# facebook/transform360

Hardware: NVIDIA H100
Metric: Mpixels/s 8K equirect->cubemap bicubic (input-plane pixels consumed per second) (higher is better)
Workload: dtype u8

## Files before the change

include/transform360_b200.h:

```cpp
#ifndef TRANSFORM360_B200_EXT_H
#define TRANSFORM360_B200_EXT_H

#include "Transform360/VideoFrameTransformHandler.h"

#ifdef __cplusplus
extern "C" {
#endif

typedef struct T360HostPlan T360HostPlan;

T360HostPlan* T360B200_hostPlanCreate(const FrameTransformContext* ctx, int inputWidth, int inputHeight,
                                      int outputWidth, int outputHeight);
#define T360_BORDER_WRAP 3
#define T360_BORDER_TRANSPARENT 5
T360HostPlan* T360B200_hostPlanCreateFromWarp(const FrameTransformContext* ctx, const float* map, int mapWidth, int mapHeight,
                                              int inputWidth, int inputHeight, int border);
void T360B200_hostPlanDestroy(T360HostPlan* plan);
int T360B200_hostPlanInfo(const T360HostPlan* plan, int info[6]);
const float* T360B200_hostPlanMap(const T360HostPlan* plan);
const int32_t* T360B200_hostPlanSamples(const T360HostPlan* plan);
int T360B200_hostPlanGather(T360HostPlan* plan, int info[10], const int32_t** jobs, const int32_t** records,
                            const uint32_t** compact);
int T360B200_hostPlanPoleCaps(T360HostPlan* plan, int info[4], const int32_t** capJobs, const uint32_t** capRecords,
                              const int32_t** launchJobs);
int T360B200_dealLanes(int interpolationAlg, int n, const int32_t* phases, int32_t* laneOf, int32_t* copyOf);
int T360B200_weightImage(int interpolationAlg, const uint8_t** image);
int T360B200_hostPlanBlurLists(T360HostPlan* const* plans, int numPlans, int width, int height, int layout[15],
                               const uint8_t** image);
int T360B200_hostPlanSegment(const T360HostPlan* plan, int i, int rect[4], int numTaps[2], const float** kx,
                             const float** ky);
int T360B200_remapTable(int interpolationAlg, const int16_t** table);

int T360B200_generateMapFromWarp(VideoFrameTransform* transform, const float* map, int mapWidth, int mapHeight, int inputWidth,
                                 int inputHeight, int border, int transformMatPlaneIndex);
int T360B200_remapFrameAsync(VideoFrameTransform* transform, int numPlanes, const float* const* deviceMaps, const int* mapPitches,
                             int border, const uint8_t* const* deviceInputs, uint8_t* const* deviceOutputs, const int* inputWidths,
                             const int* inputHeights, const int* inputPitches, const int* outputWidths, const int* outputHeights,
                             const int* outputPitches, void* cudaStream);

int T360B200_transformFramePlaneAsync(VideoFrameTransform* transform, const uint8_t* deviceInput,
                                      uint8_t* deviceOutput, int inputWidth, int inputHeight, int inputPitch,
                                      int outputWidth, int outputHeight, int outputPitch,
                                      int transformMatPlaneIndex, void* cudaStream);
int T360B200_transformFrameAsync(VideoFrameTransform* transform, int numPlanes, const uint8_t* const* deviceInputs,
                                 uint8_t* const* deviceOutputs, const int* inputWidths, const int* inputHeights,
                                 const int* inputPitches, const int* outputWidths, const int* outputHeights,
                                 const int* outputPitches, void* cudaStream);
// ... 67 lines not shown
```

profiles/trace_frame.py:

```python
#!/usr/bin/env python
import sys
from pathlib import Path

import numpy as np
import torch

sys.path.insert(0, str(Path(__file__).resolve().parents[1]))
import transform360_b200 as t360
from bench import CONFIGS
from transform360_b200 import synth
from transform360_b200.stream import FrameTransformer, StreamSpec

KINDS = {0: "class0", 1: "class1", 3: "share-stay", 4: "share", 5: "nop", 7: "seam", 8: "pole-cap", 9: "border"}


def main():
    name = sys.argv[1] if len(sys.argv) > 1 else "cfg2"
    cfg = CONFIGS[name]
    dev = torch.device("cuda", 0)
    torch.cuda.set_device(0)
    ctx = t360.make_context(**dict(cfg["ov"], enable_low_pass_filter=0))
    spec = StreamSpec(cfg["inp"][0], cfg["inp"][1], cfg["out"][0], cfg["out"][1])
    ft = FrameTransformer(ctx, spec)
    pitch = lambda w: (w + 255) // 256 * 256
    ring = 5
    d_in = [[synth.noise_plane_torch(*spec.plane_dims(p)[:2], plane=p, frame=f, device=dev, pitch=pitch(spec.plane_dims(p)[0])) for p in range(3)]
            for f in range(ring)]
    d_out = [torch.zeros((spec.plane_dims(p)[3], pitch(spec.plane_dims(p)[2])), dtype=torch.uint8, device=dev) for p in range(3)]
    calls = [ft.frame_call([(t.data_ptr(), t.stride(0)) for t in fr], [(t.data_ptr(), t.stride(0)) for t in d_out]) for fr in d_in]
    stream = torch.cuda.Stream(device=dev)
    torch.cuda.synchronize()
    for i in range(6):
        calls[i % ring](stream.cuda_stream)
    torch.cuda.synchronize()
    ft.vft.debug_trace(True)
    calls[1](stream.cuda_stream)
# ... 25 lines not shown
```

transform360_b200/csrc/gather_frame.cu:

```cuda
#include "gather_common.cuh"

#include <cuda.h>

#include <algorithm>
#include <cstring>
#include <utility>

namespace t360 {

namespace {

template <class F, int... I>
__device__ __forceinline__ void staticForImpl(F&& f, std::integer_sequence<int, I...>) {
  (f(std::integral_constant<int, I>{}), ...);
}
template <int N, class F>
__device__ __forceinline__ void staticFor(F&& f) {
  staticForImpl(f, std::make_integer_sequence<int, N>{});
}

template <int IMM>
__device__ __forceinline__ uint32_t ldsWordImm(uint32_t addr) {
  uint32_t v;
  asm volatile("ld.shared.u32 %0, [%1+%2];" : "=r"(v) : "r"(addr), "n"(IMM));
// ... 177 lines not shown
  });
}

template <int K, int PITCH, int VS>
__device__ __forceinline__ void computeTileJob(const PlaneView& pv, uint32_t stageAddr, int outX, int outY, const uint4& rec,
                                               uint32_t wAddr, int warp) {
  static_assert(PITCH % 4 == 0, "");
  const int y0 = outY + warp * kTilePatchH;
  const int dstPitch = pv.dstPitch, dstW = pv.dstW, dstH = pv.dstH;
  uint8_t* const dstRow = pv.dst + (size_t)y0 * dstPitch + outX;
  const uint32_t words[4] = {rec.x, rec.y, rec.z, rec.w};
  staticFor<kRowsPerPatchStep>([&](auto J) {
    constexpr int j = decltype(J)::value;
    const uint32_t w = words[j];
    const int col = kTilePatchW * j + ((int)(w >> 16) & (kTilePatchW - 1)), row = (int)(w >> 19) & (kTilePatchH - 1);
    if (!(w & kRecordSkip) && outX + col < dstW && y0 + row < dstH) {
      const uint32_t rowAddr = stageAddr + (w & 0x7ffcu);
      const int sh = (int)(w << 3);
      RowBytes<K> W[K];
      staticFor<K>([&](auto R) { W[decltype(R)::value] = loadRow<K, decltype(R)::value * PITCH>(rowAddr, sh); });
      const int acc = foldPixel<K, VS>(W, wAddr, (w >> 17) & kSlotFieldMask);
      dstRow[(size_t)row * dstPitch + col] = (uint8_t)biasedToByte(acc);
    }
  });
}

template <int K, int PITCH, int VS>
__device__ __forceinline__ void computeCapJob(const PlaneView& pv, uint32_t stageAddr, uint32_t recAddr, int steps, uint32_t wAddr,
                                              int warp, int lane) {
  static_assert(PITCH % 4 == 0, "");
  for (int s = warp; s < steps; s += kGroupWarps) {
    const uint2 r = ldsVec2Imm<0>(recAddr + s * kCapStepBytes + lane * 8);
    if (r.x & kRecordSkip) continue;
    const uint32_t rowAddr = stageAddr + (r.x & 0x7ffcu);
    const int sh = (int)(r.x << 3);
    RowBytes<K> W[K];
    staticFor<K>([&](auto R) { W[decltype(R)::value] = loadRow<K, decltype(R)::value * PITCH>(rowAddr, sh); });
    const int acc = foldPixel<K, VS>(W, wAddr, (r.x >> 17) & kSlotFieldMask);
    pv.dst[(size_t)(r.y >> 16) * pv.dstPitch + (r.y & 0xffffu)] = (uint8_t)biasedToByte(acc);
  }
}

template <int K, int VS>
__device__ __forceinline__ void computeBorderJob(const PlaneView& pv, uint32_t recAddr, int n, const unsigned char* wsmem, int warp, int lane) {
  SrcView sv;
  sv.bytes = pv.src;
// ... 184 lines not shown
      if constexpr (K >= 4) {
        const uint32_t mine = rec + 128 + warp * shareWarpRecordBytes(K);
        uint4 r[shareRows(K) / 8];
#pragma unroll
        for (int b = 0; b < shareRows(K) / 8; ++b) r[b] = ldsVec(mine + b * 512 + lane * 16);
        const uint32_t header = ldsWord(mine + shareRows(K) / 8 * 512 + lane * 4);
        uint8_t* dst = pv.dst + (size_t)(outY + (warp >> 1) * shareRows(K)) * pv.dstPitch + (outX + (warp & 1) * 32 + (int)(header >> kRecordColumnShift));
        if (kind == kJobShare) computeShareJob<K, stageBoxW(K, 2), VS, shareRows(K), false>(dst, pv.dstPitch, boxAddr + st * kStage, r, header, wAddr);
        else computeShareJob<K, stageBoxW(K, 2), VS, shareRows(K), true>(dst, pv.dstPitch, boxAddr + st * kStage, r, header, wAddr);
      }
    } else if (kind == kJobClass0) {
      uint4 r;
      const int quad = ((int)h.x & kJobQuadMask) - 1;
      if (quad < 0) {
        r = ldsVec(rec + 128 + warp * 512 + lane * 16);
      } else {
        r = make_uint4(kRecordSkip, kRecordSkip, kRecordSkip, kRecordSkip);
        if ((warp >> 2) == (quad >> 1)) {
          const uint2 v = ldsVec2Imm<0>(rec + 128 + (warp & 3) * 256 + lane * 8);
          if (quad & 1) { r.z = v.x; r.w = v.y; } else { r.x = v.x; r.y = v.y; }
        }
      }
      computeTileJob<K, stageBoxW(K, 0), VS>(pv, boxAddr + st * kStage, outX, outY, r, wAddr, warp);
    } else if (kind == kJobClass1) {
      computeTileJob<K, stageBoxW(K, 1), VS>(pv, boxAddr + st * kStage, outX, outY, ldsVec(rec + 128 + warp * 512 + lane * 16), wAddr, warp);
    } else if (kind == kJobSeam) {
      {
        uint4* a = reinterpret_cast<uint4*>(groupBase + st * kStage);
        const uint4* b = reinterpret_cast<const uint4*>(groupBase + (st + 1) * kStage);
        for (int i = warp * 32 + lane; i < (int)(kBox0 / 16); i += kGroupThreads) {
          uint4 x = a[i];
          const uint4 y = b[i];
          x.x |= y.x; x.y |= y.y; x.z |= y.z; x.w |= y.w;
          a[i] = x;
        }
        asm volatile("fence.proxy.async.shared::cta;" ::: "memory");
      }
      groupBarrier(group);
      computeTileJob<K, stageBoxW(K, 0), VS>(pv, boxAddr + st * kStage, outX, outY, ldsVec(rec + 128 + warp * 512 + lane * 16), wAddr, warp);
    } else if (kind == kJobCap) {
      computeCapJob<K, stageBoxW(K, 0), VS>(pv, boxAddr + st * kStage, rec + 128, (int)h.x, wAddr, warp, lane);
    } else if (kind == kJobBorder) {
      computeBorderJob<K, VS>(pv, rec + 128, (int)h.x, wsmem, warp, lane);
    }
    __syncwarp();
    if (lane == 0) mbarArrive(empty + st);
// ... 69 lines not shown
```

transform360_b200/csrc/gather_plan.cpp:

```cpp
#include "gather_plan.h"

#include <algorithm>
#include <climits>
#include <cstdint>
#include <cstring>
#include <stdexcept>
#include <thread>
#include <utility>

namespace t360 {
namespace {

template <class F>
void parallelRanges(int n, size_t workPerItem, F fn) {
  unsigned nt = std::thread::hardware_concurrency();
  if (nt == 0) nt = 1;
  if (nt > 32) nt = 32;
  if (static_cast<size_t>(n) * workPerItem < (1u << 16)) nt = 1;
  const int chunk = (n + static_cast<int>(nt) - 1) / static_cast<int>(nt);
  std::vector<std::thread> pool;
  for (unsigned t = 1; t < nt; ++t) {
    const int b = static_cast<int>(t) * chunk, e = std::min(n, b + chunk);
    if (b < e) pool.emplace_back(fn, b, e);
  }
// ... 604 lines not shown
  coverPoleCaps(h, cls, tilesX, tilesY, pixelJobs);
  for (PixelJob& pj : pixelJobs) {
    const int kind = (pj.job.outY >> kJobKindShift) & kJobKindMask;
    pj.job.recordOffset = static_cast<int>(offset / 16);
    offset += jobRecordBytes(k, kind, pj.job.outX);
    g.capJobs.push_back(pj.job);
    g.capRecords.insert(g.capRecords.end(), pj.words.begin(), pj.words.end());
    ++(kind == kJobCap ? g.numCap : g.numBorder);
  }

  std::vector<int> launch;
  for (size_t i = 0; i < g.jobs.size(); ++i)
    if (((g.jobs[i].outY >> kJobKindShift) & kJobKindMask) != kJobGeneral) launch.push_back(static_cast<int>(i));
  for (size_t i = 0; i < g.capJobs.size(); ++i) launch.push_back(-1 - static_cast<int>(i));
  auto jobOf = [&](int i) -> const GatherJob& { return i >= 0 ? g.jobs[i] : g.capJobs[-1 - i]; };
  std::stable_sort(launch.begin(), launch.end(), [&](int a, int b) { return jobLaunchRank(jobOf(a)) < jobLaunchRank(jobOf(b)); });
  for (int i : launch) {
    g.launchJobs.push_back(jobOf(i));
    g.launchNeedRows.push_back(i >= 0 ? needRows[i] : pixelJobs[-1 - i].needRows);
    g.launchRects.push_back(i >= 0 ? rects[i] : pixelJobs[-1 - i].rect);
  }
}

}
```

transform360_b200/csrc/gather_plan.h:

```cpp
#pragma once

#include <cstdint>
#include <vector>

#include "host_plan.h"
#include "kernels.cuh"

namespace t360 {

struct JobRect {
  int x0, y0, x1, y1;
};

struct GatherPlan {
  int tilesPerRow = 0, tileRows = 0, tileH = 0;
  std::vector<int2> records;
  std::vector<GatherJob> jobs;
  std::vector<uint32_t> compact;
  std::vector<GatherJob> capJobs;
  std::vector<uint32_t> capRecords;
  std::vector<GatherJob> launchJobs;
  std::vector<int> launchNeedRows;
  std::vector<JobRect> launchRects;
  int numStaged[2] = {}, numSeam = 0, numGeneral = 0, numShare = 0, numCap = 0, numBorder = 0;
  int totalStaged() const { return numSeam + numShare + numStaged[0] + numStaged[1] + numCap; }
};

void buildGatherPlan(const HostPlan& h, bool stageTiles, GatherPlan& g);

inline int jobLaunchRank(const GatherJob& job) {
  switch ((job.outY >> kJobKindShift) & kJobKindMask) {
    case kJobBorder: case kJobGeneral: return 0;
    case kJobSeam: return 1;
    case kJobClass1: return 2;
    case kJobCap: return 3;
    case kJobShareStay: return 4;
    case kJobShare: return 5;
    default: return (job.outX & kJobQuadMask) ? 7 : 6;
  }
}


int dealLanes(int k, int copies, int n, const int* slot, int* laneOf, int* copyOf);

std::vector<uint8_t> buildWeightImage(int k, const int16_t* table);

}
```

transform360_b200/csrc/kernels.cuh:

```cuda
#pragma once

#include <cuda_runtime.h>

#include <cstdint>

#include "flat_view.h"
#include "oriented_view.h"

namespace t360 {

struct GatherParams {
  const uint8_t* src;
  int srcW, srcH, srcPitch;
  uint8_t* dst;
  int dstW, dstH, dstPitch;
  const int2* samples;
  int tilesPerRow;
  const int16_t* weights;
  int kernelSize;
  int transparent;
};

struct GatherJob {
  int outX, outY;
  int boxXY;
  int recordOffset;
};
constexpr int kBoxVariants = 3;
__host__ __device__ constexpr int jobBoxField(int boxX, int boxY, int variant) { return boxX | (boxY << 16) | variant; }
__host__ __device__ constexpr int jobBoxX(int boxXY) { return boxXY & 0xfff0; }
__host__ __device__ constexpr int jobBoxY(int boxXY) { return (int)((unsigned)boxXY >> 16); }
__host__ __device__ constexpr int jobBoxVariant(int boxXY) { return boxXY & 15; }
using StagedTile = GatherJob;
constexpr int kJobClass0 = 0, kJobClass1 = 1, kJobGeneral = 2, kJobShareStay = 3, kJobShare = 4, kJobNop = 5, kJobExit = 6, kJobSeam = 7,
              kJobCap = 8, kJobBorder = 9;
constexpr int kJobQuadMask = 7;
constexpr uint32_t kRecordSkip = 0x8000u;
constexpr int kJobKindShift = 24, kJobRowMask = (1 << kJobKindShift) - 1;
constexpr int kJobPlaneShift = 28, kJobKindMask = (1 << (kJobPlaneShift - kJobKindShift)) - 1;

constexpr int kGroupThreads = 256, kGroupWarps = kGroupThreads / 32;
__host__ __device__ constexpr int gatherGroups(int k) { return k == 8 ? 2 : 3; }
#ifndef T360_CLAIM_BATCH
#define T360_CLAIM_BATCH 1
#endif
constexpr int kClaimBatch = T360_CLAIM_BATCH;
constexpr int kGatherTileW = 32, kFrameTileH = 32;
constexpr int kTilePatchW = 8, kTilePatchH = 4, kRowsPerPatchStep = 4;
constexpr int kShareW = 64;
__host__ __device__ constexpr int shareRows(int ) { return 8; }
__host__ __device__ constexpr int shareH(int k) { return 4 * shareRows(k); }
constexpr int kNumBoxClasses = 3;
__host__ __device__ constexpr int boxClassOf(int kind) { return (kind == kJobShare || kind == kJobShareStay) ? 2 : (kind == kJobClass1 ? 1 : 0); }
__host__ __device__ constexpr int stageBoxW(int , int cls) { return cls == 2 ? 192 : (cls == 0 ? 208 : 240); }
__host__ __device__ constexpr int stageBoxH(int k, int cls) {
  return k == 8 ? (cls == 2 ? 80 : (cls == 0 ? 72 : 128)) : (cls == 2 ? 72 : (cls == 0 ? 64 : 96));
}
__host__ __device__ constexpr int boxVariantRows(int k, int cls, int v) {
// ... 28 lines not shown
  return weightDiagonal(k) ? (slotFieldValue ^ (vector * kDiagonalStep)) : slotFieldValue + vector * weightVectorStride(k, copies);
}
__host__ __device__ constexpr int weightBankGroups(int k) { return k == 2 ? 16 : 8; }
__host__ __device__ constexpr int weightLanesPerPass(int k) { return k == 2 ? 16 : 8; }

__host__ __device__ constexpr int shareWarpRecordBytes(int k) { return shareRows(k) / 8 * 32 * 16 + 32 * 4; }
__host__ __device__ constexpr int shareJobRecordBytes(int k) { return kGroupWarps * shareWarpRecordBytes(k); }
constexpr int kTileJobRecordBytes = kGroupWarps * 32 * 16;
constexpr int kQuadJobRecordBytes = kGroupWarps / 2 * 32 * 8;
__host__ __device__ constexpr int tileJobRecordBytes(int outXField) { return (outXField & kJobQuadMask) ? kQuadJobRecordBytes : kTileJobRecordBytes; }
__host__ __device__ constexpr int stageRecordBytes(int k) {
  return 128 + (shareJobRecordBytes(k) > kTileJobRecordBytes ? shareJobRecordBytes(k) : kTileJobRecordBytes);
}
constexpr int kCapStepBytes = 32 * 8, kBorderPixelBytes = 16;
__host__ __device__ constexpr int capJobMaxSteps(int k) { return (stageRecordBytes(k) - 128) / kCapStepBytes; }
__host__ __device__ constexpr int borderJobMaxPixels(int k) { return (stageRecordBytes(k) - 128) / kBorderPixelBytes; }
__host__ __device__ constexpr int jobRecordBytes(int k, int kind, int outXField) {
  return kind == kJobShare || kind == kJobShareStay ? shareJobRecordBytes(k)
         : kind == kJobCap                          ? outXField * kCapStepBytes
         : kind == kJobBorder                       ? outXField * kBorderPixelBytes
                                                    : tileJobRecordBytes(outXField);
}
constexpr int kRecordColumnShift = 27;

constexpr int kMaxFramePlanes = 3;
struct PlaneView {
  const uint8_t* src;
  uint8_t* dst;
  const uint4* records;
  int srcW, srcH, srcPitch;
  int dstW, dstH, dstPitch;
};
struct FrameGatherParams {
  PlaneView plane[kMaxFramePlanes];
  const uint4* weightImage;
  int kernelSize, numPlanes;
};

__host__ __device__ constexpr int gatherThreads(int k) { return k == 8 ? 512 : 256; }
__host__ __device__ constexpr int gatherTileH(int k) { return gatherThreads(k) / 32 * 4; }

struct StagedParams {
  const GatherJob* tiles;
  int numTiles;
  int* claimCounter;
  unsigned long long* trace;
// ... 152 lines not shown
```

transform360_b200/csrc/video_frame_transform.cpp:

```cpp
#include <cuda.h>
#include <cuda_runtime.h>

#include <algorithm>
#include <chrono>
#include <climits>
#include <cmath>
#include <condition_variable>
#include <cstdarg>
#include <cstdio>
#include <cstdlib>
#include <cstring>
#include <map>
#include <memory>
#include <mutex>
#include <new>
#include <shared_mutex>
#include <stdexcept>
#include <string>
#include <string_view>
#include <thread>
#include <vector>

#include "host_plan.h"
#include "gather_plan.h"
// ... 1325 lines not shown
    std::lock_guard<std::mutex> lock(lazyMu_);
    auto& buf = weights_[k];
    if (!buf.ptr) {
      buf.reserve(static_cast<size_t>(1024) * k * k);
      CU(cudaMemcpy(buf.ptr, host, buf.bytes(), cudaMemcpyHostToDevice));
      const std::vector<uint8_t> image = t360::buildWeightImage(k, host);
      weightImages_[k].reserve(image.size());
      CU(cudaMemcpy(weightImages_[k].ptr, image.data(), image.size(), cudaMemcpyHostToDevice));
    }
    return buf.ptr;
  }

  DevicePlan upload(HostIndexPlan& p, const FrameTransformContext& ctx) {
    const HostPlan& h = p.host;
    DevicePlan d;
    d.inW = h.inW; d.inH = h.inH; d.outW = h.outW; d.outH = h.outH; d.mapW = h.mapW; d.mapH = h.mapH;
    d.kernelSize = h.kernelSize;
    d.transparent = h.transparentBorder;
    d.warp = h.warp;
    d.stereoFormat = ctx.input_stereo_format;
    if (d.kernelSize > 0) {
      deviceWeights(ctx.interpolation_alg);
      t360::GatherPlan& g = p.gather;
      d.tilesPerRow = g.tilesPerRow;
      d.samples.reserve(g.records.size());
      CU(cudaMemcpy(d.samples.ptr, g.records.data(), g.records.size() * sizeof(int2), cudaMemcpyHostToDevice));
      d.numStaged = g.totalStaged();
      d.numBorder = g.numBorder;
      d.numJobs = static_cast<int>(g.launchJobs.size());
      if (!g.launchJobs.empty()) {
        d.gatherJobs.reserve(g.launchJobs.size());
        CU(cudaMemcpy(d.gatherJobs.ptr, g.launchJobs.data(), g.launchJobs.size() * sizeof(GatherJob), cudaMemcpyHostToDevice));
      }
      if (!g.compact.empty() || !g.capRecords.empty()) {
        d.records.reserve(g.compact.size() + g.capRecords.size());
        if (!g.compact.empty())
          CU(cudaMemcpy(d.records.ptr, g.compact.data(), g.compact.size() * sizeof(uint32_t), cudaMemcpyHostToDevice));
        if (!g.capRecords.empty())
          CU(cudaMemcpy(d.records.ptr + g.compact.size(), g.capRecords.data(), g.capRecords.size() * sizeof(uint32_t), cudaMemcpyHostToDevice));
      }
      d.hostJobs = std::move(g.launchJobs);
      d.jobNeedRows = std::move(g.launchNeedRows);
      d.jobRects = std::move(g.launchRects);
    }
    d.lowPass = ctx.enable_low_pass_filter != 0;
    if (d.lowPass) {
// ... 696 lines not shown
}

T360_API int T360B200_generateMapFromWarp(VideoFrameTransform* t, const float* map, int mapW, int mapH, int inW, int inH, int border,
                                          int planIndex) {
  if (!t) return 0;
  return t->generateMapFromWarp(map, mapW, mapH, inW, inH, border, planIndex);
}

T360_API int VideoFrameTransform_transformFramePlane(VideoFrameTransform* transform, uint8_t* inputData,
                                                     uint8_t* outputData, int inputWidth, int inputHeight,
                                                     int inputWidthWithPadding, int outputWidth, int outputHeight,
                                                     int outputWidthWithPadding, int transformMatPlaneIndex,
                                                     int imagePlaneIndex) {
  if (!transform) return 0;
  return transform->transformFramePlane(inputData, outputData, inputWidth, inputHeight, inputWidthWithPadding,
                                        outputWidth, outputHeight, outputWidthWithPadding, transformMatPlaneIndex,
                                        imagePlaneIndex);
}

struct T360HostPlan {
  HostPlan plan;
  t360::GatherPlan gather;
  bool gatherBuilt = false;
  std::vector<uint8_t> blurImage;
};

T360_API T360HostPlan* T360B200_hostPlanCreate(const FrameTransformContext* ctx, int inW, int inH, int outW, int outH) {
  if (!ctx) return nullptr;
  std::unique_ptr<T360HostPlan> p(new (std::nothrow) T360HostPlan);
  if (!p) return nullptr;
  try {
    if (!t360::buildHostPlan(*ctx, inW, inH, outW, outH, p->plan)) return nullptr;
  } catch (const std::exception& ex) {
    std::printf("Could not build the host plan. Error: %s\n", ex.what());
    return nullptr;
  }
  return p.release();
}
T360_API T360HostPlan* T360B200_hostPlanCreateFromWarp(const FrameTransformContext* ctx, const float* map, int mapW, int mapH, int inW,
                                                       int inH, int border) {
  if (!ctx) return nullptr;
  std::unique_ptr<T360HostPlan> p(new (std::nothrow) T360HostPlan);
  if (!p) return nullptr;
  try {
    if (!t360::buildWarpHostPlan(*ctx, map, mapW, mapH, inW, inH, border, p->plan)) return nullptr;
  } catch (const std::exception& ex) {
// ... 27 lines not shown
  } catch (const std::exception& ex) {
    std::printf("Could not build the gather plan. Error: %s\n", ex.what());
    return 0;
  }
  const t360::GatherPlan& g = plan->gather;
  info[0] = g.tilesPerRow; info[1] = g.tileRows; info[2] = g.tileH; info[3] = static_cast<int>(g.jobs.size());
  info[4] = g.numStaged[0]; info[5] = g.numStaged[1]; info[6] = g.numSeam; info[7] = g.numGeneral;
  info[8] = g.numShare; info[9] = static_cast<int>(g.compact.size());
  if (jobs) *jobs = g.jobs.empty() ? nullptr : reinterpret_cast<const int32_t*>(g.jobs.data());
  if (records) *records = reinterpret_cast<const int32_t*>(g.records.data());
  if (compact) *compact = g.compact.empty() ? nullptr : g.compact.data();
  return 1;
}
T360_API int T360B200_hostPlanPoleCaps(T360HostPlan* plan, int info[4], const int32_t** capJobs, const uint32_t** capRecords,
                                       const int32_t** launchJobs) {
  int gatherInfo[10];
  if (!plan || !info || !T360B200_hostPlanGather(plan, gatherInfo, nullptr, nullptr, nullptr)) return 0;
  const t360::GatherPlan& g = plan->gather;
  info[0] = g.numCap; info[1] = g.numBorder; info[2] = static_cast<int>(g.capRecords.size());
  info[3] = static_cast<int>(g.launchJobs.size());
  if (capJobs) *capJobs = g.capJobs.empty() ? nullptr : reinterpret_cast<const int32_t*>(g.capJobs.data());
  if (capRecords) *capRecords = g.capRecords.empty() ? nullptr : g.capRecords.data();
  if (launchJobs) *launchJobs = g.launchJobs.empty() ? nullptr : reinterpret_cast<const int32_t*>(g.launchJobs.data());
  return 1;
}
T360_API int T360B200_hostPlanBlurLists(T360HostPlan* const* plans, int numPlans, int width, int height, int layout[15],
                                        const uint8_t** image) {
  if (!plans || numPlans < 1 || numPlans > t360::kMaxFramePlanes || !layout || !image) return 0;
  for (int p = 0; p < numPlans; ++p)
    if (!plans[p]) return 0;
  try {
    t360::BlurLists lists[t360::kMaxFramePlanes];
    const t360::BlurLists* planes[t360::kMaxFramePlanes];
    bool clear = false;
    for (int p = 0; p < numPlans; ++p) {
      const HostPlan& h = plans[p]->plan;
      bool c = false;
      t360::buildBlurLists(h.segments, h.taps, width > 0 ? width : h.inW, height > 0 ? height : h.inH, h.ctx.input_stereo_format, lists[p], &c);
      clear = clear || c;
      planes[p] = &lists[p];
    }
    std::vector<uint8_t>& img = plans[0]->blurImage;
    img.clear();
    const t360::BlurLayout l = t360::packBlurLists(numPlans > 1 ? t360::mergeBlurLists(planes, numPlans) : lists[0], img, img);
    const long long v[15] = {l.numStrips[0], l.numStrips[1], l.numStrips[2], l.numTiles, l.numDirect, l.numTaps, l.tileSmem, clear,
                             static_cast<long long>(l.stripAt[0]), static_cast<long long>(l.stripAt[1]), static_cast<long long>(l.stripAt[2]),
// ... 218 lines not shown
```

transform360_b200/handler.py:

```python
from __future__ import annotations

import ctypes as C
import os
from pathlib import Path

import numpy as np

PKG = Path(__file__).resolve().parent
LIB_PATH = PKG / "lib" / "libTransform360.so"

LAYOUT_CUBEMAP_32, LAYOUT_CUBEMAP_23_OFFCENTER, LAYOUT_FLAT_FIXED, LAYOUT_EQUIRECT = 0, 1, 2, 3
LAYOUT_BARREL, LAYOUT_BARREL_SPLIT, LAYOUT_EAC_32, LAYOUT_N = 4, 5, 6, 7
STEREO_FORMAT_TB, STEREO_FORMAT_LR, STEREO_FORMAT_MONO, STEREO_FORMAT_GUESS, STEREO_FORMAT_N = 0, 1, 2, 3, 4
NEAREST, LINEAR, CUBIC, LANCZOS4 = 0, 1, 2, 4
BORDER_WRAP, BORDER_TRANSPARENT = 3, 5


def _warp_map(map) -> np.ndarray:
    m = np.ascontiguousarray(map, np.float32)
    if m.ndim != 3 or m.shape[2] != 2:
        raise ValueError(f"a warp map is float32 [h][w][2] (x, y per output pixel), got shape {m.shape}")
    return m


# ... 114 lines not shown
    L.T360B200_hostPlanCreate.argtypes = [C.POINTER(FrameTransformContext)] + [ci] * 4
    L.T360B200_hostPlanCreateFromWarp.restype = vp
    L.T360B200_hostPlanCreateFromWarp.argtypes = [C.POINTER(FrameTransformContext), vp] + [ci] * 5
    L.T360B200_generateMapFromWarp.restype = ci
    L.T360B200_generateMapFromWarp.argtypes = [vp, vp] + [ci] * 6
    L.T360B200_remapFrameAsync.restype = ci
    L.T360B200_remapFrameAsync.argtypes = [vp, ci, vp, vp, ci] + [vp] * 8 + [vp]
    L.T360B200_hostPlanDestroy.restype = None
    L.T360B200_hostPlanDestroy.argtypes = [vp]
    L.T360B200_hostPlanInfo.restype = ci
    L.T360B200_hostPlanInfo.argtypes = [vp, C.POINTER(ci)]
    L.T360B200_hostPlanMap.restype = vp
    L.T360B200_hostPlanMap.argtypes = [vp]
    L.T360B200_hostPlanSamples.restype = vp
    L.T360B200_hostPlanSamples.argtypes = [vp]
    L.T360B200_hostPlanSegment.restype = ci
    L.T360B200_hostPlanSegment.argtypes = [vp, ci, C.POINTER(ci), C.POINTER(ci), C.POINTER(vp), C.POINTER(vp)]
    L.T360B200_hostPlanGather.restype = ci
    L.T360B200_hostPlanGather.argtypes = [vp, C.POINTER(ci), C.POINTER(vp), C.POINTER(vp), C.POINTER(vp)]
    L.T360B200_hostPlanPoleCaps.restype = ci
    L.T360B200_hostPlanBlurLists.restype = ci
    L.T360B200_hostPlanBlurLists.argtypes = [vp, ci, ci, ci, C.POINTER(ci), C.POINTER(vp)]
    L.T360B200_hostPlanPoleCaps.argtypes = [vp, C.POINTER(ci), C.POINTER(vp), C.POINTER(vp), C.POINTER(vp)]
    L.T360B200_weightImage.restype = ci
    L.T360B200_weightImage.argtypes = [ci, C.POINTER(vp)]
    L.T360B200_remapTable.restype = ci
    L.T360B200_remapTable.argtypes = [ci, C.POINTER(vp)]
    L.T360B200_transformFramePlaneAsync.restype = ci
    L.T360B200_transformFramePlaneAsync.argtypes = [vp, vp, vp] + [ci] * 7 + [vp]
    L.T360B200_transformFrameAsync.restype = ci
    L.T360B200_transformFrameAsync.argtypes = [vp, ci, vp, vp] + [vp] * 6 + [vp]
    L.T360B200_lowPassPlaneAsync.restype = ci
    L.T360B200_lowPassPlaneAsync.argtypes = [vp, vp, vp] + [ci] * 5 + [vp]
    L.T360B200_reconfigure.restype = ci
    L.T360B200_reconfigure.argtypes = [vp, C.POINTER(FrameTransformContext)]
    L.T360B200_reconfigureAsync.restype = ci
    L.T360B200_reconfigureAsync.argtypes = [vp, C.POINTER(FrameTransformContext)]
    L.T360B200_reconfigureWait.restype = ci
    L.T360B200_reconfigureWait.argtypes = [vp, ci]
    L.T360B200_transformFrameViewAsync.restype = ci
    L.T360B200_transformFrameViewAsync.argtypes = [vp, C.POINTER(T360View), ci, vp, vp] + [vp] * 6 + [vp]
    L.T360B200_viewSamples.restype = ci
    L.T360B200_viewSamples.argtypes = [C.POINTER(FrameTransformContext), C.POINTER(T360View)] + [ci] * 4 + [vp]
    L.T360B200_transformFrameOrientedAsync.restype = ci
    L.T360B200_transformFrameOrientedAsync.argtypes = [vp, C.POINTER(T360Orientation), ci, vp, vp] + [vp] * 6 + [vp]
    L.T360B200_orientedSamples.restype = ci
# ... 13 lines not shown
    L.T360B200_debugTraceRead.restype = C.c_ulonglong
    L.T360B200_debugTraceRead.argtypes = [vp, vp, C.c_ulonglong]
    L.T360B200_synchronize.restype = ci
    L.T360B200_synchronize.argtypes = [vp]
    L.T360B200_stream.restype = vp
    L.T360B200_stream.argtypes = [vp]
    L.T360B200_kernelLaunchCount.restype = C.c_ulonglong
    L.T360B200_planDeviceBytes.restype = C.c_ulonglong
    L.T360B200_planDeviceBytes.argtypes = [vp, ci]
    L.T360B200_planTileCounts.restype = ci
    L.T360B200_planTileCounts.argtypes = [vp, ci, C.POINTER(ci)]
    L.T360B200_deviceCount.restype = ci
    L.T360B200_version.restype = C.c_char_p
    if path is None:
        _lib = L
    return L


EXPORTED_SYMBOLS = [
    "VideoFrameTransform_new", "VideoFrameTransform_delete", "VideoFrameTransform_generateMapForPlane",
    "VideoFrameTransform_transformFramePlane", "T360B200_hostPlanCreate", "T360B200_hostPlanCreateFromWarp", "T360B200_hostPlanDestroy",
    "T360B200_generateMapFromWarp", "T360B200_remapFrameAsync",
    "T360B200_hostPlanInfo", "T360B200_hostPlanMap", "T360B200_hostPlanSamples", "T360B200_hostPlanSegment",
    "T360B200_hostPlanGather", "T360B200_hostPlanPoleCaps", "T360B200_hostPlanBlurLists", "T360B200_weightImage", "T360B200_dealLanes",
    "T360B200_remapTable", "T360B200_transformFramePlaneAsync", "T360B200_transformFrameAsync",
    "T360B200_lowPassPlaneAsync", "T360B200_reconfigure", "T360B200_reconfigureAsync", "T360B200_reconfigureWait",
    "T360B200_transformFrameViewAsync", "T360B200_viewSamples",
    "T360B200_transformFrameOrientedAsync", "T360B200_orientedSamples", "T360B200_transformFramePoseAsync", "T360B200_poseSamples",
    "T360B200_lensMap", "T360B200_transformFrameLensAsync",
    "T360B200_setPinHostPlanes", "T360B200_debugTrace", "T360B200_debugTraceRead", "T360B200_synchronize", "T360B200_stream", "T360B200_kernelLaunchCount", "T360B200_planDeviceBytes",
    "T360B200_planTileCounts", "T360B200_deviceCount", "T360B200_version",
]


class VideoFrameTransform:

    def __init__(self, ctx: FrameTransformContext):
        self._lib = load()
        self.ctx = ctx
        self._h = self._lib.VideoFrameTransform_new(C.byref(ctx))
        if not self._h:
            raise MemoryError("VideoFrameTransform_new returned NULL")

    def close(self):
        if getattr(self, "_h", None):
            self._lib.VideoFrameTransform_delete(self._h)
            self._h = None
# ... 186 lines not shown
        if not self._lib.T360B200_hostPlanGather(self._h, info, C.byref(jobs), C.byref(recs), C.byref(comp)):
            raise ValueError("T360B200_hostPlanGather failed")
        tpr, trows, th, nj = info[0], info[1], info[2], info[3]
        n = tpr * trows * th * 32 * 2
        records = np.frombuffer((C.c_int32 * n).from_address(recs.value), np.int32).reshape(tpr * trows, th, 32, 2).copy()
        j = compact = None
        if nj and jobs.value:
            j = np.frombuffer((C.c_int32 * (nj * 4)).from_address(jobs.value), np.int32).reshape(nj, 4).copy()
        if info[9] and comp.value:
            compact = np.frombuffer((C.c_uint32 * info[9]).from_address(comp.value), np.uint32).copy()
        return dict(tiles_per_row=tpr, tile_rows=trows, tile_h=th, jobs=j, records=records, compact=compact,
                    counts=dict(class0=info[4], class1=info[5], seam=info[6], general=info[7], share=info[8]))

    def pole_caps(self):
        info = (C.c_int * 4)()
        jobs, recs, launch = C.c_void_p(), C.c_void_p(), C.c_void_p()
        if not self._lib.T360B200_hostPlanPoleCaps(self._h, info, C.byref(jobs), C.byref(recs), C.byref(launch)):
            raise ValueError("T360B200_hostPlanPoleCaps failed")
        n, m = info[0] + info[1], info[3]
        as_jobs = lambda p, k: np.frombuffer((C.c_int32 * (k * 4)).from_address(p.value), np.int32).reshape(k, 4).copy() if k and p.value else np.zeros((0, 4), np.int32)
        records = np.frombuffer((C.c_uint32 * info[2]).from_address(recs.value), np.uint32).copy() if info[2] and recs.value else np.zeros(0, np.uint32)
        return dict(counts=dict(cap=info[0], border=info[1]), jobs=as_jobs(jobs, n), records=records, launch=as_jobs(launch, m))

    def blur_lists(self, *others, width=0, height=0):
        plans = (C.c_void_p * (1 + len(others)))(self._h, *[o._h for o in others])
        lay, img = (C.c_int * 15)(), C.c_void_p()
        if not self._lib.T360B200_hostPlanBlurLists(plans, len(plans), width, height, lay, C.byref(img)):
            raise ValueError("T360B200_hostPlanBlurLists failed (message on stdout)")
        image = C.string_at(img.value, lay[14]) if lay[14] else b""
        arr = lambda at, n, cols, dt: np.frombuffer(image, dt, n * cols, at).reshape(n, cols).copy()
        return dict(image=image, strips=[arr(lay[8 + c], lay[c], 9, np.int32) for c in range(3)], tiles=arr(lay[11], lay[3], 8, np.int32),
                    direct=arr(lay[12], lay[4], 8, np.int32), taps=np.frombuffer(image, np.float32, lay[5], lay[13]).copy(),
                    offsets=list(lay[8:14]), tile_smem=lay[6], needs_clear=bool(lay[7]))

    def segments(self):
        out = []
        rect, nk = (C.c_int * 4)(), (C.c_int * 2)()
        kx, ky = C.c_void_p(), C.c_void_p()
        for i in range(self.num_segments):
            assert self._lib.T360B200_hostPlanSegment(self._h, i, rect, nk, C.byref(kx), C.byref(ky))
            a = np.frombuffer((C.c_float * nk[0]).from_address(kx.value), np.float32).copy()
            b = np.frombuffer((C.c_float * nk[1]).from_address(ky.value), np.float32).copy()
            out.append((rect[0], rect[1], rect[2], rect[3], a, b))
        return out


# ... 57 lines not shown
```

Measured before the change: 720,900.

## Add tile-walk job kind reusing bicubic tap words across output rows

Adds a new job kind for bicubic class-0 tiles. Each lane keeps its 4x2 shared-memory tap words in registers across the four output rows of a patch step and reloads only the words that change: a row step, a left or right word shift, or a full reload. The host planner encodes these per-lane walk flags into the records. It also picks a lane-dealing row and weight-copy assignment that minimise a modelled count of shared-memory bank wavefronts. This cuts shared-memory loads and bank conflicts in the gather kernel, at the cost of more register pressure, extra branching and heavier plan-build work on the host.

Result: faster. 764,500, median of 6 (+6.0%).

```diff
diff --git a/include/transform360_b200.h b/include/transform360_b200.h
--- a/include/transform360_b200.h
+++ b/include/transform360_b200.h
@@ -23,6 +23,8 @@
                             const uint32_t** compact);
 int T360B200_hostPlanPoleCaps(T360HostPlan* plan, int info[4], const int32_t** capJobs, const uint32_t** capRecords,
                               const int32_t** launchJobs);
+int T360B200_hostPlanTileWalk(T360HostPlan* plan, int info[4], long long model[4], const int32_t** launchJobs,
+                              const uint32_t** records);
 int T360B200_dealLanes(int interpolationAlg, int n, const int32_t* phases, int32_t* laneOf, int32_t* copyOf);
 int T360B200_weightImage(int interpolationAlg, const uint8_t** image);
 int T360B200_hostPlanBlurLists(T360HostPlan* const* plans, int numPlans, int width, int height, int layout[15],
diff --git a/profiles/trace_frame.py b/profiles/trace_frame.py
--- a/profiles/trace_frame.py
+++ b/profiles/trace_frame.py
@@ -11,7 +11,7 @@
 from transform360_b200 import synth
 from transform360_b200.stream import FrameTransformer, StreamSpec
 
-KINDS = {0: "class0", 1: "class1", 3: "share-stay", 4: "share", 5: "nop", 7: "seam", 8: "pole-cap", 9: "border"}
+KINDS = {0: "class0", 1: "class1", 3: "share-stay", 4: "share", 5: "nop", 7: "seam", 8: "pole-cap", 9: "border", 10: "tile-walk"}
 
 
 def main():
diff --git a/transform360_b200/csrc/gather_frame.cu b/transform360_b200/csrc/gather_frame.cu
--- a/transform360_b200/csrc/gather_frame.cu
+++ b/transform360_b200/csrc/gather_frame.cu
@@ -223,6 +223,50 @@
       const int acc = foldPixel<K, VS>(W, wAddr, (w >> 17) & kSlotFieldMask);
       dstRow[(size_t)row * dstPitch + col] = (uint8_t)biasedToByte(acc);
     }
+  });
+}
+
+template <int PITCH, int VS>
+__device__ __forceinline__ void computeWalkJob(const PlaneView& pv, uint32_t stageAddr, int outX, int outY, const uint4& rec,
+                                               uint32_t wAddr, int warp) {
+  constexpr int K = 4;
+  static_assert(PITCH % 4 == 0, "");
+  const uint32_t words[4] = {rec.x, rec.y, rec.z, rec.w};
+  uint8_t* const dst = pv.dst + (size_t)(outY + warp * kTilePatchH) * pv.dstPitch + outX + ((int)(words[0] >> 16) & 31);
+  uint32_t q0[K], q1[K];
+  {
+    const uint32_t a = stageAddr + (words[0] & 0x7ffcu);
+    staticFor<K>([&](auto R) {
+      constexpr int r = decltype(R)::value;
+      q0[r] = ldsWordImm<r * PITCH>(a);
+      q1[r] = ldsWordImm<r * PITCH + 4>(a);
+    });
+  }
+  staticFor<kRowsPerPatchStep>([&](auto J) {
+    constexpr int j = decltype(J)::value;
+    const uint32_t w = words[j];
+    if constexpr (j > 0) {
+      const uint32_t a = stageAddr + (w & 0x7ffcu);
+      const bool step = (w & kWalkRowStep) != 0, right = (w & kWalkWordRight) != 0, left = (w & kWalkWordLeft) != 0,
+                 reload = (w & kWalkReload) != 0;
+      staticFor<K>([&](auto R) {
+        constexpr int r = decltype(R)::value;
+        const uint32_t o0 = (r + 1 < K && step) ? q0[r + 1 < K ? r + 1 : r] : q0[r];
+        const uint32_t o1 = (r + 1 < K && step) ? q1[r + 1 < K ? r + 1 : r] : q1[r];
+        const bool enter = reload || (r == K - 1 && step);
+        uint32_t n0 = right ? o1 : o0, n1 = left ? o0 : o1;
+        if (enter || left) n0 = ldsWordImm<r * PITCH>(a);
+        if (enter || right) n1 = ldsWordImm<r * PITCH + 4>(a);
+        q0[r] = n0;
+        q1[r] = n1;
+      });
+    }
+    const int sh = (int)(w << 3);
+    RowBytes<K> W[K];
+#pragma unroll
+    for (int r = 0; r < K; ++r) W[r].b[0] = __funnelshift_r(q0[r], q1[r], sh);
+    const int acc = foldPixel<K, VS>(W, wAddr, (w >> 17) & kSlotFieldMask);
+    dst[(size_t)j * pv.dstPitch] = (uint8_t)biasedToByte(acc);
   });
 }
 
@@ -453,6 +497,9 @@
         }
       }
       computeTileJob<K, stageBoxW(K, 0), VS>(pv, boxAddr + st * kStage, outX, outY, r, wAddr, warp);
+    } else if (kind == kJobWalk) {
+      if constexpr (K == 4)
+        computeWalkJob<stageBoxW(K, 0), VS>(pv, boxAddr + st * kStage, outX, outY, ldsVec(rec + 128 + warp * 512 + lane * 16), wAddr, warp);
     } else if (kind == kJobClass1) {
       computeTileJob<K, stageBoxW(K, 1), VS>(pv, boxAddr + st * kStage, outX, outY, ldsVec(rec + 128 + warp * 512 + lane * 16), wAddr, warp);
     } else if (kind == kJobSeam) {
diff --git a/transform360_b200/csrc/gather_plan.cpp b/transform360_b200/csrc/gather_plan.cpp
--- a/transform360_b200/csrc/gather_plan.cpp
+++ b/transform360_b200/csrc/gather_plan.cpp
@@ -650,4 +650,186 @@
   }
 }
 
-}
+namespace {
+
+int wordWavefronts(const int* word, const bool* active) {
+  int v[32], n = 0, perBank[32] = {}, worst = 0;
+  for (int i = 0; i < 32; ++i)
+    if (active[i]) v[n++] = word[i];
+  std::sort(v, v + n);
+  for (int i = 0; i < n; ++i)
+    if (i == 0 || v[i] != v[i - 1]) worst = std::max(worst, ++perBank[v[i] & 31]);
+  return worst;
+}
+int vectorWavefronts(const uint32_t* field) {
+  int cost = 0;
+  for (int q = 0; q < 4; ++q) {
+    int worst = 0;
+    for (int i = 8 * q; i < 8 * q + 8; ++i) {
+      int distinct = 0;
+      for (int j = 8 * q; j < 8 * q + 8; ++j) {
+        if (((field[j] >> 4) & 7) != ((field[i] >> 4) & 7)) continue;
+        bool first = true;
+        for (int m = 8 * q; m < j && first; ++m) first = field[m] != field[j];
+        distinct += first;
+      }
+      worst = std::max(worst, distinct);
+    }
+    cost += worst;
+  }
+  return cost;
+}
+
+constexpr int kWalkPitch = 208;
+static_assert(kWalkPitch == stageBoxW(4, 0), "");
+
+void walkWarp(const HostPlan& h, int x0, int y0, int boxX, int boxY, int w, int dealt, uint32_t* words, TileWalkStats& cost) {
+  const int k = 4, copies = weightCopies(k), rowWords = kWalkPitch / 4;
+  int slot[32], laneOf[32], copyOf[32];
+  for (int c = 0; c < 32; ++c) slot[c] = weightSlotOf(k, h.samples[static_cast<size_t>(y0 + 4 * w + dealt) * h.mapW + x0 + c].rowPhase & 1023);
+  dealLanes(k, copies, 32, slot, laneOf, copyOf);
+  int prevRow[32], prevWord[32];
+  for (int j = 0; j < kRowsPerPatchStep; ++j) {
+    const SamplePoint* row = &h.samples[static_cast<size_t>(y0 + 4 * w + j) * h.mapW + x0];
+    int rowOf[32], wordOf[32], off[32], s[32];
+    uint32_t flags[32];
+    for (int c = 0; c < 32; ++c) {
+      const int lane = laneOf[c];
+      rowOf[lane] = (row[c].rowPhase >> 10) - boxY;
+      off[lane] = rowOf[lane] * kWalkPitch + (row[c].col0 - boxX);
+      wordOf[lane] = off[lane] >> 2;
+      s[lane] = weightSlotOf(k, row[c].rowPhase & 1023);
+      flags[lane] = static_cast<uint32_t>(c) << 16;
+      if (j > 0) {
+        const int dy = rowOf[lane] - prevRow[lane], da = (wordOf[lane] - rowOf[lane] * rowWords) - (prevWord[lane] - prevRow[lane] * rowWords);
+        flags[lane] = dy < 0 || dy > 1 || da < -1 || da > 1
+                          ? kWalkReload
+                          : (dy ? kWalkRowStep : 0u) | (da > 0 ? kWalkWordRight : 0u) | (da < 0 ? kWalkWordLeft : 0u);
+      }
+    }
+    uint32_t field[32];
+    for (int lane = 0; lane < 32; ++lane) {
+      int c = 0;
+      while (laneOf[c] != lane) ++c;
+      field[lane] = slotField(k, row[c].rowPhase & 1023, copyOf[c]);
+    }
+    if (j != dealt)
+      for (int q = 0; q < 4; ++q) {
+        int load[8] = {};
+        for (int lane = 8 * q; lane < 8 * q + 8; ++lane) {
+          uint32_t best = 0;
+          int bestLoad = INT_MAX;
+          for (int cp = 0; cp < copies; ++cp) {
+            const uint32_t cand = static_cast<uint32_t>((weightSlotInCopy(s[lane], cp) << 4) | (cp << 14));
+            bool shared = false;
+            for (int m = 8 * q; m < lane; ++m) shared = shared || field[m] == cand;
+            const int l = shared ? -1 : load[(cand >> 4) & 7];
+            if (l < bestLoad) { bestLoad = l; best = cand; }
+          }
+          field[lane] = best;
+          if (bestLoad >= 0) ++load[(best >> 4) & 7];
+        }
+      }
+    if (j == 0) {
+      bool all[32];
+      std::fill(all, all + 32, true);
+      for (int r = 0; r < k; ++r)
+        for (int e = 0; e < 2; ++e) {
+          int a[32];
+          for (int lane = 0; lane < 32; ++lane) a[lane] = wordOf[lane] + r * rowWords + e;
+          cost.walkTaps += wordWavefronts(a, all);
+        }
+    } else {
+      for (int r = 0; r < k; ++r)
+        for (int e = 0; e < 2; ++e) {
+          int a[32];
+          bool active[32];
+          for (int lane = 0; lane < 32; ++lane) {
+            const uint32_t f = flags[lane];
+            const bool enter = (f & kWalkReload) || (r == k - 1 && (f & kWalkRowStep));
+            active[lane] = enter || (f & (e == 0 ? kWalkWordLeft : kWalkWordRight));
+            a[lane] = wordOf[lane] + r * rowWords + e;
+          }
+          cost.walkTaps += wordWavefronts(a, active);
+        }
+    }
+    cost.walkWeights += 2 * vectorWavefronts(field);
+    for (int lane = 0; lane < 32; ++lane) {
+      words[lane * 4 + j] = static_cast<uint32_t>(off[lane]) | flags[lane] | (field[lane] << 17);
+      prevRow[lane] = rowOf[lane];
+      prevWord[lane] = wordOf[lane];
+    }
+  }
+}
+
+void walkTile(const HostPlan& h, const GatherJob& job, const uint32_t* tileWords, uint32_t* walkWords, TileWalkStats& cost) {
+  const int k = 4;
+  const int x0 = job.outX & ~kJobQuadMask, y0 = job.outY & kJobRowMask, boxX = jobBoxX(job.boxXY), boxY = jobBoxY(job.boxXY);
+  const int rowWords = kWalkPitch / 4;
+  for (int w = 0; w < kGroupWarps; ++w) {
+    for (int j = 0; j < kRowsPerPatchStep; ++j) {
+      int word[32];
+      bool active[32];
+      uint32_t field[32];
+      for (int lane = 0; lane < 32; ++lane) {
+        const uint32_t v = tileWords[w * 128 + lane * 4 + j];
+        word[lane] = static_cast<int>(v & 0x7fffu) >> 2;
+        active[lane] = true;
+        field[lane] = (v >> 17) & kSlotFieldMask;
+      }
+      for (int r = 0; r < k; ++r)
+        for (int e = 0; e < 2; ++e) {
+          int a[32];
+          for (int lane = 0; lane < 32; ++lane) a[lane] = word[lane] + r * rowWords + e;
+          cost.patchTaps += wordWavefronts(a, active);
+        }
+      cost.patchWeights += 2 * vectorWavefronts(field);
+    }
+    TileWalkStats best;
+    for (int dealt = 0; dealt < kRowsPerPatchStep; ++dealt) {
+      TileWalkStats c;
+      uint32_t words[128];
+      walkWarp(h, x0, y0, boxX, boxY, w, dealt, words, c);
+      if (dealt == 0 || c.walkTaps + c.walkWeights < best.walkTaps + best.walkWeights) {
+        best = c;
+        std::copy(words, words + 128, walkWords + w * 128);
+      }
+    }
+    cost.walkTaps += best.walkTaps;
+    cost.walkWeights += best.walkWeights;
+  }
+}
+
+}
+
+TileWalkStats applyTileWalk(const HostPlan& h, GatherPlan& g) {
+  TileWalkStats total;
+  if (h.kernelSize != 4) return total;
+  std::vector<int> tiles;
+  for (size_t i = 0; i < g.launchJobs.size(); ++i) {
+    const GatherJob& job = g.launchJobs[i];
+    const int x0 = job.outX & ~kJobQuadMask, y0 = job.outY & kJobRowMask;
+    if (((job.outY >> kJobKindShift) & kJobKindMask) == kJobClass0 && (job.outX & kJobQuadMask) == 0 &&
+        x0 + kGatherTileW <= h.mapW && y0 + kFrameTileH <= h.mapH)
+      tiles.push_back(static_cast<int>(i));
+  }
+  std::vector<TileWalkStats> cost(tiles.size());
+  parallelRanges(static_cast<int>(tiles.size()), 1 << 16, [&](int begin, int end) {
+    std::vector<uint32_t> walk(kTileJobRecordBytes / 4);
+    for (int i = begin; i < end; ++i) {
+      GatherJob& job = g.launchJobs[tiles[i]];
+      uint32_t* words = g.compact.data() + static_cast<size_t>(job.recordOffset) * 4;
+      walkTile(h, job, words, walk.data(), cost[i]);
+      std::copy(walk.begin(), walk.end(), words);
+      job.outY = (job.outY & ~(kJobKindMask << kJobKindShift)) | (kJobWalk << kJobKindShift);
+    }
+  });
+  total.tiles = static_cast<int>(tiles.size());
+  for (const TileWalkStats& c : cost) {
+    total.patchTaps += c.patchTaps; total.patchWeights += c.patchWeights;
+    total.walkTaps += c.walkTaps; total.walkWeights += c.walkWeights;
+  }
+  return total;
+}
+
+}
diff --git a/transform360_b200/csrc/gather_plan.h b/transform360_b200/csrc/gather_plan.h
--- a/transform360_b200/csrc/gather_plan.h
+++ b/transform360_b200/csrc/gather_plan.h
@@ -36,10 +36,17 @@
     case kJobCap: return 3;
     case kJobShareStay: return 4;
     case kJobShare: return 5;
+    case kJobWalk: return 6;
     default: return (job.outX & kJobQuadMask) ? 7 : 6;
   }
 }
 
+
+struct TileWalkStats {
+  int tiles = 0;
+  long long patchTaps = 0, patchWeights = 0, walkTaps = 0, walkWeights = 0;
+};
+TileWalkStats applyTileWalk(const HostPlan& h, GatherPlan& g);
 
 int dealLanes(int k, int copies, int n, const int* slot, int* laneOf, int* copyOf);
 
diff --git a/transform360_b200/csrc/kernels.cuh b/transform360_b200/csrc/kernels.cuh
--- a/transform360_b200/csrc/kernels.cuh
+++ b/transform360_b200/csrc/kernels.cuh
@@ -33,7 +33,7 @@
 __host__ __device__ constexpr int jobBoxVariant(int boxXY) { return boxXY & 15; }
 using StagedTile = GatherJob;
 constexpr int kJobClass0 = 0, kJobClass1 = 1, kJobGeneral = 2, kJobShareStay = 3, kJobShare = 4, kJobNop = 5, kJobExit = 6, kJobSeam = 7,
-              kJobCap = 8, kJobBorder = 9;
+              kJobCap = 8, kJobBorder = 9, kJobWalk = 10;
 constexpr int kJobQuadMask = 7;
 constexpr uint32_t kRecordSkip = 0x8000u;
 constexpr int kJobKindShift = 24, kJobRowMask = (1 << kJobKindShift) - 1;
@@ -108,6 +108,7 @@
                                                     : tileJobRecordBytes(outXField);
 }
 constexpr int kRecordColumnShift = 27;
+constexpr uint32_t kWalkRowStep = 1u << 15, kWalkWordRight = 1u << 16, kWalkWordLeft = 1u << 17, kWalkReload = 1u << 18;
 
 constexpr int kMaxFramePlanes = 3;
 struct PlaneView {
diff --git a/transform360_b200/csrc/video_frame_transform.cpp b/transform360_b200/csrc/video_frame_transform.cpp
--- a/transform360_b200/csrc/video_frame_transform.cpp
+++ b/transform360_b200/csrc/video_frame_transform.cpp
@@ -1371,6 +1371,7 @@
     if (d.kernelSize > 0) {
       deviceWeights(ctx.interpolation_alg);
       t360::GatherPlan& g = p.gather;
+      t360::applyTileWalk(h, g);
       d.tilesPerRow = g.tilesPerRow;
       d.samples.reserve(g.records.size());
       CU(cudaMemcpy(d.samples.ptr, g.records.data(), g.records.size() * sizeof(int2), cudaMemcpyHostToDevice));
@@ -2113,6 +2114,10 @@
   HostPlan plan;
   t360::GatherPlan gather;
   bool gatherBuilt = false;
+  t360::GatherPlan device;
+  t360::TileWalkStats walk;
+  std::vector<uint32_t> deviceRecords;
+  bool deviceBuilt = false;
   std::vector<uint8_t> blurImage;
 };
 
@@ -2186,6 +2191,28 @@
   if (capJobs) *capJobs = g.capJobs.empty() ? nullptr : reinterpret_cast<const int32_t*>(g.capJobs.data());
   if (capRecords) *capRecords = g.capRecords.empty() ? nullptr : g.capRecords.data();
   if (launchJobs) *launchJobs = g.launchJobs.empty() ? nullptr : reinterpret_cast<const int32_t*>(g.launchJobs.data());
+  return 1;
+}
+T360_API int T360B200_hostPlanTileWalk(T360HostPlan* plan, int info[4], long long model[4], const int32_t** launchJobs,
+                                       const uint32_t** records) {
+  int gatherInfo[10];
+  if (!plan || !info || !T360B200_hostPlanGather(plan, gatherInfo, nullptr, nullptr, nullptr)) return 0;
+  if (!plan->deviceBuilt) {
+    plan->device = plan->gather;
+    plan->walk = t360::applyTileWalk(plan->plan, plan->device);
+    plan->deviceRecords = plan->device.compact;
+    plan->deviceRecords.insert(plan->deviceRecords.end(), plan->device.capRecords.begin(), plan->device.capRecords.end());
+    plan->deviceBuilt = true;
+  }
+  const t360::GatherPlan& g = plan->device;
+  info[0] = static_cast<int>(g.launchJobs.size()); info[1] = static_cast<int>(plan->deviceRecords.size());
+  info[2] = plan->walk.tiles; info[3] = 0;
+  if (model) {
+    model[0] = plan->walk.patchTaps; model[1] = plan->walk.patchWeights;
+    model[2] = plan->walk.walkTaps; model[3] = plan->walk.walkWeights;
+  }
+  if (launchJobs) *launchJobs = g.launchJobs.empty() ? nullptr : reinterpret_cast<const int32_t*>(g.launchJobs.data());
+  if (records) *records = plan->deviceRecords.empty() ? nullptr : plan->deviceRecords.data();
   return 1;
 }
 T360_API int T360B200_hostPlanBlurLists(T360HostPlan* const* plans, int numPlans, int width, int height, int layout[15],
diff --git a/transform360_b200/handler.py b/transform360_b200/handler.py
--- a/transform360_b200/handler.py
+++ b/transform360_b200/handler.py
@@ -160,6 +160,8 @@
     L.T360B200_hostPlanBlurLists.restype = ci
     L.T360B200_hostPlanBlurLists.argtypes = [vp, ci, ci, ci, C.POINTER(ci), C.POINTER(vp)]
     L.T360B200_hostPlanPoleCaps.argtypes = [vp, C.POINTER(ci), C.POINTER(vp), C.POINTER(vp), C.POINTER(vp)]
+    L.T360B200_hostPlanTileWalk.restype = ci
+    L.T360B200_hostPlanTileWalk.argtypes = [vp, C.POINTER(ci), C.POINTER(C.c_longlong), C.POINTER(vp), C.POINTER(vp)]
     L.T360B200_weightImage.restype = ci
     L.T360B200_weightImage.argtypes = [ci, C.POINTER(vp)]
     L.T360B200_remapTable.restype = ci
@@ -219,7 +221,7 @@
     "VideoFrameTransform_transformFramePlane", "T360B200_hostPlanCreate", "T360B200_hostPlanCreateFromWarp", "T360B200_hostPlanDestroy",
     "T360B200_generateMapFromWarp", "T360B200_remapFrameAsync",
     "T360B200_hostPlanInfo", "T360B200_hostPlanMap", "T360B200_hostPlanSamples", "T360B200_hostPlanSegment",
-    "T360B200_hostPlanGather", "T360B200_hostPlanPoleCaps", "T360B200_hostPlanBlurLists", "T360B200_weightImage", "T360B200_dealLanes",
+    "T360B200_hostPlanGather", "T360B200_hostPlanPoleCaps", "T360B200_hostPlanTileWalk", "T360B200_hostPlanBlurLists", "T360B200_weightImage", "T360B200_dealLanes",
     "T360B200_remapTable", "T360B200_transformFramePlaneAsync", "T360B200_transformFrameAsync",
     "T360B200_lowPassPlaneAsync", "T360B200_reconfigure", "T360B200_reconfigureAsync", "T360B200_reconfigureWait",
     "T360B200_transformFrameViewAsync", "T360B200_viewSamples",
@@ -452,6 +454,17 @@
         records = np.frombuffer((C.c_uint32 * info[2]).from_address(recs.value), np.uint32).copy() if info[2] and recs.value else np.zeros(0, np.uint32)
         return dict(counts=dict(cap=info[0], border=info[1]), jobs=as_jobs(jobs, n), records=records, launch=as_jobs(launch, m))
 
+    def tile_walk(self):
+        info, model = (C.c_int * 4)(), (C.c_longlong * 4)()
+        launch, recs = C.c_void_p(), C.c_void_p()
+        if not self._lib.T360B200_hostPlanTileWalk(self._h, info, model, C.byref(launch), C.byref(recs)):
+            raise ValueError("T360B200_hostPlanTileWalk failed")
+        m, n = info[0], info[1]
+        jobs = np.frombuffer((C.c_int32 * (m * 4)).from_address(launch.value), np.int32).reshape(m, 4).copy() if m and launch.value else np.zeros((0, 4), np.int32)
+        records = np.frombuffer((C.c_uint32 * n).from_address(recs.value), np.uint32).copy() if n and recs.value else np.zeros(0, np.uint32)
+        return dict(launch=jobs, records=records, walks=info[2],
+                    model=dict(zip(("tile_taps", "tile_weights", "walk_taps", "walk_weights"), list(model))))
+
     def blur_lists(self, *others, width=0, height=0):
         plans = (C.c_void_p * (1 + len(others)))(self._h, *[o._h for o in others])
         lay, img = (C.c_int * 15)(), C.c_void_p()
```
